# sujeetv/parquet-go

Measured on AMD Instinct MI355X. Metric: decoded GB/s (uncompressed output) per GPU & node at 1/2/4/8; % HBM roofline, higher is better.
Workload: dtype int32; 1 GPU; C2: optional INT32, 100000000 rows x 7 dictionary widths (b=1,2,4,8,12,16,20), ~10% nulls, RLE_DICTIONARY (uniform indices), V1, UNCOMPRESSED, 20000 rows/page; bytes_in=821696760, bytes_out=3220121800, streams=2, parallelism=single GPU

## Files before the change

### parquet-go_amd/csrc/pqg_lev1.h

```cpp
#pragma once
#include "pqg_levdec.h"

namespace pqg {

constexpr int kL1MaxN = 4096;
constexpr int kL1MaxCount = 32768 - 16;
constexpr int kL1Win = kL1MaxN + 64;
constexpr uint32_t kL1Far = 254, kL1Bad = 255;

struct Lev1Shared {
  uint8_t win[kL1Win];
  uint32_t tab[kL1MaxN / 4 + 2];
};

struct L1Hdr {
  uint32_t nx;
  uint32_t cnt;
  uint32_t pay;
  bool bp, bad;
};

__device__ __forceinline__ L1Hdr l1_hdr(uint32_t lo, uint32_t hi, uint32_t q, uint32_t n) {
  const uint32_t cont = ~lo & 0x80808080u;
  const uint32_t hl = (cont ? (uint32_t)__builtin_ctz(cont) >> 3 : 4u) + 1;
  const uint32_t hf = (lo & 0x7f) | ((lo >> 1) & 0x3f80) | ((lo >> 2) & 0x1fc000) | ((lo >> 3) & 0xfe00000);
  const uint32_t h = __builtin_amdgcn_ubfe(hf, 0, 7 * hl);
  const uint32_t g = h >> 1;
  const bool bp = (h & 1) != 0;
  const uint32_t vb = (uint32_t)((((uint64_t)hi << 32) | lo) >> (8 * hl)) & 0xff;
  const uint32_t ve = q + hl;
  L1Hdr r;
  r.bp = bp;
  r.bad = (hl > 4) | (ve > n) | (g == 0) | (!bp & ((ve >= n) | (vb > 1)));
  r.cnt = bp ? g * 8 : g;
  r.pay = bp ? ve : vb;
  r.nx = ve + (bp ? g : 1u);
  return r;
}
__device__ __forceinline__ L1Hdr l1_parse(const PQG_L uint8_t* win, uint32_t mis, uint32_t q, uint32_t n) {
  const uint32_t wo = mis + q;
  const PQG_L uint32_t* d = (const PQG_L uint32_t*)(win + (wo & ~3u));
  const uint32_t a = d[0], b = d[1], c = d[2];
  const uint32_t sft = (wo & 3) * 8;
  return l1_hdr(__builtin_amdgcn_alignbit(b, a, sft), __builtin_amdgcn_alignbit(c, b, sft), q, n);
}
struct L1Run {
  uint32_t hl, g, vb;
  bool bp;
};
__device__ __forceinline__ L1Run l1_run(const PQG_L uint8_t* win, uint32_t mis, uint32_t q) {
  const uint32_t wo = mis + q;
  const PQG_L uint32_t* d = (const PQG_L uint32_t*)(win + (wo & ~3u));
  const uint32_t a = d[0], b = d[1], c = d[2];
  const uint32_t sft = (wo & 3) * 8;
  const uint32_t lo = __builtin_amdgcn_alignbit(b, a, sft), hi = __builtin_amdgcn_alignbit(c, b, sft);
  const uint32_t cont = ~lo & 0x80808080u;
  L1Run r;
  r.hl = (cont ? (uint32_t)__builtin_ctz(cont) >> 3 : 3u) + 1;
  const uint32_t hf = (lo & 0x7f) | ((lo >> 1) & 0x3f80) | ((lo >> 2) & 0x1fc000) | ((lo >> 3) & 0xfe00000);
  const uint32_t h = __builtin_amdgcn_ubfe(hf, 0, 7 * r.hl);
  r.g = h >> 1;
  r.bp = (h & 1) != 0;
  r.vb = (uint32_t)((((uint64_t)hi << 32) | lo) >> (8 * r.hl)) & 0xff;
  return r;
}

__device__ __forceinline__ uint32_t l1_code(const L1Hdr& h, uint32_t e) {
  const uint32_t d = h.nx - e;
  return h.bad ? kL1Bad : (d < kL1Far ? d : kL1Far);
}

__device__ __forceinline__ void l1_or_run(PQG_L uint32_t* bm, const PQG_L uint32_t* W, uint32_t s, uint32_t len,
                                          bool bp, uint32_t sbit) {
  const uint32_t e = s + len;
  for (uint32_t k = s >> 5; 32 * k < e; k++) {
    const uint32_t lo = s > 32 * k ? s : 32 * k;
    const uint32_t hi = e < 32 * k + 32 ? e : 32 * k + 32;
    const uint32_t cnt = hi - lo;
    const uint32_t m = cnt >= 32 ? 0xffffffffu : ((1u << cnt) - 1);
    uint32_t v = m;
    if (bp) {
      const uint32_t sb = sbit + (lo - s);
      v = __builtin_amdgcn_alignbit(W[(sb >> 5) + 1], W[sb >> 5], sb & 31) & m;
    }
    v <<= (lo - 32 * k);
    if (v) __hip_atomic_fetch_or(bm + k, v, __ATOMIC_RELAXED, __HIP_MEMORY_SCOPE_WAVEFRONT);
  }
}

__device__ __forceinline__ bool lev1_page(gcu8 p, uint32_t n, uint32_t count, gu8 out, Lev1Shared& sh, uint32_t* nn_out) {
  const int lane = lane_id();
  if (n == 0 || n > (uint32_t)kL1MaxN || count > (uint32_t)kL1MaxCount) return false;
  PQG_L uint8_t* win = lds_ptr(sh.win);
  PQG_T(t0);
  const uintptr_t pa = (uintptr_t)p;
  const uint32_t mis = (uint32_t)(pa & 15);
  const uintptr_t base = pa - mis;
  const uint32_t lim = mis + n;
  constexpr int kR = (kL1Win + 1023) / 1024;
  uint4 v[kR];
#pragma unroll
  for (int h = 0; h < kR; h++) {
    const uint32_t g = 1024u * h + 16u * lane;
    v[h] = ldg16(g < lim ? base + g : base);
  }
#pragma unroll
  for (int h = 0; h < kR; h++) {
    const uint32_t g = 1024u * h + 16u * lane;
    if (g < (uint32_t)kL1Win) sts16(win + g, g < lim ? mask_tail(v[h], g, lim) : make_uint4(0, 0, 0, 0));
  }
  __builtin_amdgcn_wave_barrier();
  PQG_T(t1);
  PQG_ACC(20, t0, t1);
  PQG_L uint8_t* T = (PQG_L uint8_t*)lds_ptr(sh.tab);
  const uint32_t S = (((n + 63) >> 6) + 3) & ~3u;
  const uint32_t a = (uint32_t)lane * S;
  const uint32_t e = a + S < n ? a + S : n;
  int q = (int)e - 1;
  for (int r = (int)((e > a ? e - a : 0u) & 3); r > 0; r--, q--) {
    const L1Hdr h = l1_parse(win, mis, (uint32_t)q, n);
    uint32_t code = l1_code(h, e);
    if (!h.bad && h.nx < e) code = T[h.nx];
    T[q] = (uint8_t)code;
  }
  for (; q >= (int)a + 3; q -= 4) {
    const uint32_t q0 = (uint32_t)q - 3;
    const uint32_t wo = mis + q0;
    const PQG_L uint32_t* d = (const PQG_L uint32_t*)(win + (wo & ~3u));
    const uint32_t d0 = d[0], d1 = d[1], d2 = d[2], d3 = d[3];
    const uint32_t o = wo & 3;
    L1Hdr h[4];
#pragma unroll
    for (int j = 0; j < 4; j++) {
      const uint32_t oj = o + j;
      const uint32_t sft = (oj & 3) * 8;
      const bool up = oj >= 4;
      const uint32_t x0 = up ? d1 : d0, x1 = up ? d2 : d1, x2 = up ? d3 : d2;
      h[j] = l1_hdr(__builtin_amdgcn_alignbit(x1, x0, sft), __builtin_amdgcn_alignbit(x2, x1, sft), q0 + j, n);
    }
    uint32_t t[4], c[4];
    bool in[4];
#pragma unroll
    for (int j = 0; j < 4; j++) {
      in[j] = !h[j].bad & (h[j].nx < e);
      t[j] = T[in[j] ? h[j].nx : q0 + 3];
      c[j] = l1_code(h[j], e);
    }
    const uint32_t c3 = in[3] ? t[3] : c[3];
    const uint32_t c2 = in[2] ? t[2] : c[2];
    const uint32_t c1 = in[1] ? (h[1].nx == q0 + 3 ? c3 : t[1]) : c[1];
    const uint32_t c0 = in[0] ? (h[0].nx == q0 + 3 ? c3 : h[0].nx == q0 + 2 ? c2 : t[0]) : c[0];
    *(PQG_L uint32_t*)(T + q0) = c0 | c1 << 8 | c2 << 16 | c3 << 24;
  }
  __builtin_amdgcn_wave_barrier();
  PQG_T(t2);
  PQG_ACC(21, t1, t2);
  uint32_t E = 0, myE = 0;
  bool ok = true;
  for (int l = 0; l < 64; l++) {
    const uint32_t al = (uint32_t)l * S;
    if (lane == l) myE = E;
    if (al >= n) continue;
    const uint32_t el = al + S < n ? al + S : n;
    if (E >= el) continue;
    const uint32_t code = (uint32_t)__builtin_amdgcn_readfirstlane((int)T[E]);
    if (code == kL1Bad) { ok = false; break; }
    if (code == kL1Far) {
      uint32_t q = E;
      while (q < el) {
        const L1Hdr h = l1_parse(win, mis, q, n);
        if (h.bad) { ok = false; break; }
        q = (uint32_t)__builtin_amdgcn_readfirstlane((int)h.nx);
      }
      if (!ok) break;
      E = q;
    } else {
      E = el + code;
    }
  }
  PQG_T(t3);
  PQG_ACC(22, t2, t3);
  if (!ok) { PQG_ACC(27, 0, 1); return false; }
#ifdef PQG_L1_STOP_AFTER_LINK
  *nn_out = 0;
  return true;
#endif
  uint32_t C = 0;
  uint64_t cm = 0;
  for (uint32_t q = myE; q < e;) {
    const L1Run r = l1_run(win, mis, q);
    const uint32_t cnt = r.bp ? r.g * 8 : r.g;
    C = C + cnt < (1u << 24) ? C + cnt : (1u << 24);
    cm |= 1ull << (q - a);
    q += r.hl + (r.bp ? r.g : 1u);
  }
  const uint32_t incl = ldpp_incl_add_sat(C);
  const uint32_t total = (uint32_t)__builtin_amdgcn_readlane((int)incl, 63);
  if (total < count) return false;
  const uint32_t B = incl - C;
  PQG_T(t4);
  PQG_ACC(23, t3, t4);
  const uintptr_t oa = (uintptr_t)out;
  const uintptr_t a0 = oa & ~(uintptr_t)15;
  const uint32_t pre = (uint32_t)(oa - a0);
  const uint32_t end = pre + count;
  PQG_L uint32_t* bm = lds_ptr(sh.tab);
  const uint32_t nw = (end + 31) >> 5;
  __builtin_amdgcn_wave_barrier();
  for (uint32_t k = (uint32_t)lane; k <= nw; k += 64) bm[k] = 0u;
  __builtin_amdgcn_wave_barrier();
  const PQG_L uint32_t* W = (const PQG_L uint32_t*)win;
  bool fail = false;
  uint32_t c = B;
  uint32_t k = (pre + c) >> 5, fill = (pre + c) & 31;
  uint64_t acc = 0;
  const uint32_t kfirst = k;
  uint32_t nn = 0;
  uint64_t m = c < count ? cm : 0ull;
#ifdef PQG_L1_SKIP_EMIT
  m = 0;
#endif
  auto flush = [&](uint32_t word) {
    if (k == kfirst) __hip_atomic_fetch_or(bm + k, word, __ATOMIC_RELAXED, __HIP_MEMORY_SCOPE_WAVEFRONT);
    else bm[k] = word;
    nn += __builtin_popcount(word);
    k++;
  };
  uint32_t rq = 0;
  L1Run r{};
  if (m) {
    rq = a + (uint32_t)__builtin_ctzll(m);
    m &= m - 1;
    r = l1_run(win, mis, rq);
  }
  bool more = c < count && cm != 0;
  while (more) {
    const L1Run cur = r;
    const uint32_t cq = rq;
    const bool next = m != 0;
    if (next) {
      rq = a + (uint32_t)__builtin_ctzll(m);
      m &= m - 1;
      r = l1_run(win, mis, rq);
    }
    const uint32_t cnt = cur.bp ? cur.g * 8 : cur.g;
    uint32_t take = cnt < count - c ? cnt : count - c;
    const uint32_t pay = cq + cur.hl;
    if (cur.bp && pay + ((take + 7) >> 3) - 1 >= n) { fail = true; break; }
    c += take;
    const uint32_t pat = cur.vb ? 0xffffffffu : 0u;
    const bool bp = cur.bp;
    uint32_t sb = bp ? (mis + pay) * 8 : 0u;
    while (take) {
      const uint32_t nb = take < 32 ? take : 32;
      const uint32_t src = __builtin_amdgcn_alignbit(W[(sb >> 5) + 1], W[sb >> 5], sb & 31);
      const uint32_t bits = (bp ? src : pat) & (nb >= 32 ? 0xffffffffu : ((1u << nb) - 1));
      acc |= (uint64_t)bits << fill;
      fill += nb;
      take -= nb;
      sb += nb;
      if (fill >= 32) {
        flush((uint32_t)acc);
        acc >>= 32;
        fill -= 32;
      }
    }
    more = next && c < count;
  }
  if (fill) {
    __hip_atomic_fetch_or(bm + k, (uint32_t)acc, __ATOMIC_RELAXED, __HIP_MEMORY_SCOPE_WAVEFRONT);
    nn += __builtin_popcount((uint32_t)acc);
  }
  if (__ballot(fail)) return false;
  PQG_T(t5);
  PQG_ACC(24, t4, t5);
  __builtin_amdgcn_wave_barrier();
  const PQG_L uint16_t* B16 = (const PQG_L uint16_t*)lds_ptr(sh.tab);
#ifdef PQG_L1_SKIP_EXPAND
  const uint32_t g0 = 1, g1 = 0;
#else
  const uint32_t g0 = (pre + 15) >> 4, g1 = end >> 4;
#endif
  for (uint32_t g = g0 + (uint32_t)lane; g < g1; g += 64) {
    const uint32_t b16 = B16[g];
    uint32_t wv[4];
#pragma unroll
    for (int j = 0; j < 4; j++) wv[j] = (((b16 >> (4 * j)) & 0xfu) * 0x00204081u) & 0x01010101u;
    stg16o(a0 + 16 * g, make_uint4(wv[0], wv[1], wv[2], wv[3]));
  }
  if (lane < 32) {
    const uint32_t gr = lane < 16 ? (pre >> 4) : (end >> 4);
    const uint32_t i = 16 * gr + (uint32_t)(lane & 15);
    if (i >= pre && i < end && (i < 16 * g0 || i >= 16 * g1))
      *(PQG_G uint8_t*)(a0 + i) = (uint8_t)((B16[gr] >> (lane & 15)) & 1);
  }
  *nn_out = (uint32_t)wave_sum((int64_t)nn);
  PQG_T(t6);
  PQG_ACC(25, t5, t6);
  PQG_ACC(26, 0, 1);
  return true;
}

}
```

Baseline: 1428 GB/s.

## SWAR-parse four RLE level headers per word and flatten emit loop

Replaces the four per-byte level header parses in the backward jump-table pass with a SIMD-within-a-register routine. It decodes four candidate headers at once from packed bytes, derives their lengths, bad/far flags and codes with byte-lane arithmetic, and treats headers longer than two bytes as 'far' for the slow path. It also flattens the nested run/chunk loops of the bitmap emit phase into a single loop that refills runs on demand, and moves the parser into a shared host/device header. The aim is fewer ALU ops and less branch divergence in definition-level decoding, at the cost of more intricate bit logic and extra tail handling near the page end.

```diff
diff --git a/parquet-go_amd/csrc/pqg_lev1.h b/parquet-go_amd/csrc/pqg_lev1.h
--- a/parquet-go_amd/csrc/pqg_lev1.h
+++ b/parquet-go_amd/csrc/pqg_lev1.h
@@ -1,42 +1,18 @@
 #pragma once
 #include "pqg_levdec.h"
+#include "pqg_lev1_parse.h"
 
 namespace pqg {
 
 constexpr int kL1MaxN = 4096;
 constexpr int kL1MaxCount = 32768 - 16;
 constexpr int kL1Win = kL1MaxN + 64;
-constexpr uint32_t kL1Far = 254, kL1Bad = 255;
 
 struct Lev1Shared {
   uint8_t win[kL1Win];
   uint32_t tab[kL1MaxN / 4 + 2];
 };
 
-struct L1Hdr {
-  uint32_t nx;
-  uint32_t cnt;
-  uint32_t pay;
-  bool bp, bad;
-};
-
-__device__ __forceinline__ L1Hdr l1_hdr(uint32_t lo, uint32_t hi, uint32_t q, uint32_t n) {
-  const uint32_t cont = ~lo & 0x80808080u;
-  const uint32_t hl = (cont ? (uint32_t)__builtin_ctz(cont) >> 3 : 4u) + 1;
-  const uint32_t hf = (lo & 0x7f) | ((lo >> 1) & 0x3f80) | ((lo >> 2) & 0x1fc000) | ((lo >> 3) & 0xfe00000);
-  const uint32_t h = __builtin_amdgcn_ubfe(hf, 0, 7 * hl);
-  const uint32_t g = h >> 1;
-  const bool bp = (h & 1) != 0;
-  const uint32_t vb = (uint32_t)((((uint64_t)hi << 32) | lo) >> (8 * hl)) & 0xff;
-  const uint32_t ve = q + hl;
-  L1Hdr r;
-  r.bp = bp;
-  r.bad = (hl > 4) | (ve > n) | (g == 0) | (!bp & ((ve >= n) | (vb > 1)));
-  r.cnt = bp ? g * 8 : g;
-  r.pay = bp ? ve : vb;
-  r.nx = ve + (bp ? g : 1u);
-  return r;
-}
 __device__ __forceinline__ L1Hdr l1_parse(const PQG_L uint8_t* win, uint32_t mis, uint32_t q, uint32_t n) {
   const uint32_t wo = mis + q;
   const PQG_L uint32_t* d = (const PQG_L uint32_t*)(win + (wo & ~3u));
@@ -70,24 +46,6 @@
   return h.bad ? kL1Bad : (d < kL1Far ? d : kL1Far);
 }
 
-__device__ __forceinline__ void l1_or_run(PQG_L uint32_t* bm, const PQG_L uint32_t* W, uint32_t s, uint32_t len,
-                                          bool bp, uint32_t sbit) {
-  const uint32_t e = s + len;
-  for (uint32_t k = s >> 5; 32 * k < e; k++) {
-    const uint32_t lo = s > 32 * k ? s : 32 * k;
-    const uint32_t hi = e < 32 * k + 32 ? e : 32 * k + 32;
-    const uint32_t cnt = hi - lo;
-    const uint32_t m = cnt >= 32 ? 0xffffffffu : ((1u << cnt) - 1);
-    uint32_t v = m;
-    if (bp) {
-      const uint32_t sb = sbit + (lo - s);
-      v = __builtin_amdgcn_alignbit(W[(sb >> 5) + 1], W[sb >> 5], sb & 31) & m;
-    }
-    v <<= (lo - 32 * k);
-    if (v) __hip_atomic_fetch_or(bm + k, v, __ATOMIC_RELAXED, __HIP_MEMORY_SCOPE_WAVEFRONT);
-  }
-}
-
 __device__ __forceinline__ bool lev1_page(gcu8 p, uint32_t n, uint32_t count, gu8 out, Lev1Shared& sh, uint32_t* nn_out) {
   const int lane = lane_id();
   if (n == 0 || n > (uint32_t)kL1MaxN || count > (uint32_t)kL1MaxCount) return false;
@@ -117,7 +75,11 @@
   const uint32_t a = (uint32_t)lane * S;
   const uint32_t e = a + S < n ? a + S : n;
   int q = (int)e - 1;
-  for (int r = (int)((e > a ? e - a : 0u) & 3); r > 0; r--, q--) {
+  const uint32_t len = e > a ? e - a : 0u;
+  uint32_t top = len & 3;
+  if (e - top + 3 > n) top += 4;
+  top = top < len ? top : len;
+  for (int r = (int)top; r > 0; r--, q--) {
     const L1Hdr h = l1_parse(win, mis, (uint32_t)q, n);
     uint32_t code = l1_code(h, e);
     if (!h.bad && h.nx < e) code = T[h.nx];
@@ -127,30 +89,24 @@
     const uint32_t q0 = (uint32_t)q - 3;
     const uint32_t wo = mis + q0;
     const PQG_L uint32_t* d = (const PQG_L uint32_t*)(win + (wo & ~3u));
-    const uint32_t d0 = d[0], d1 = d[1], d2 = d[2], d3 = d[3];
-    const uint32_t o = wo & 3;
-    L1Hdr h[4];
+    const uint32_t d0 = d[0], d1 = d[1], d2 = d[2];
+    const uint32_t sft = (wo & 3) * 8;
+    const uint32_t b0 = __builtin_amdgcn_alignbit(d1, d0, sft), b4 = __builtin_amdgcn_alignbit(d2, d1, sft);
+    const L1Quad h = l1_quad(b0, __builtin_amdgcn_alignbit(b4, b0, 8), __builtin_amdgcn_alignbit(b4, b0, 16));
+    const L1Codes cd = l1_quad_codes(h, e - q0);
+    const uint32_t in7 = cd.in, code = cd.code;
+    const uint32_t inm = in7 | (in7 - (in7 >> 7));
+    uint32_t nx[4], t[4];
 #pragma unroll
     for (int j = 0; j < 4; j++) {
-      const uint32_t oj = o + j;
-      const uint32_t sft = (oj & 3) * 8;
-      const bool up = oj >= 4;
-      const uint32_t x0 = up ? d1 : d0, x1 = up ? d2 : d1, x2 = up ? d3 : d2;
-      h[j] = l1_hdr(__builtin_amdgcn_alignbit(x1, x0, sft), __builtin_amdgcn_alignbit(x2, x1, sft), q0 + j, n);
-    }
-    uint32_t t[4], c[4];
-    bool in[4];
-#pragma unroll
-    for (int j = 0; j < 4; j++) {
-      in[j] = !h[j].bad & (h[j].nx < e);
-      t[j] = T[in[j] ? h[j].nx : q0 + 3];
-      c[j] = l1_code(h[j], e);
-    }
-    const uint32_t c3 = in[3] ? t[3] : c[3];
-    const uint32_t c2 = in[2] ? t[2] : c[2];
-    const uint32_t c1 = in[1] ? (h[1].nx == q0 + 3 ? c3 : t[1]) : c[1];
-    const uint32_t c0 = in[0] ? (h[0].nx == q0 + 3 ? c3 : h[0].nx == q0 + 2 ? c2 : t[0]) : c[0];
-    *(PQG_L uint32_t*)(T + q0) = c0 | c1 << 8 | c2 << 16 | c3 << 24;
+      nx[j] = q0 + j + ((h.len >> (8 * j)) & 0xff);
+      t[j] = T[(in7 >> (8 * j + 7)) & 1 ? nx[j] : q0 + 3];
+    }
+    const uint32_t up = (code & ~inm) | ((t[2] << 16 | t[3] << 24) & inm);
+    const uint32_t c3 = up >> 24, c2 = (up >> 16) & 0xff;
+    const uint32_t t1 = nx[1] == q0 + 3 ? c3 : t[1];
+    const uint32_t t0 = nx[0] == q0 + 3 ? c3 : nx[0] == q0 + 2 ? c2 : t[0];
+    *(PQG_L uint32_t*)(T + q0) = up | ((t0 | t1 << 8) & inm);
   }
   __builtin_amdgcn_wave_barrier();
   PQG_T(t2);
@@ -228,46 +184,45 @@
   };
   uint32_t rq = 0;
   L1Run r{};
-  if (m) {
+  bool have = m != 0;
+  if (have) {
     rq = a + (uint32_t)__builtin_ctzll(m);
     m &= m - 1;
     r = l1_run(win, mis, rq);
   }
-  bool more = c < count && cm != 0;
-  while (more) {
-    const L1Run cur = r;
-    const uint32_t cq = rq;
-    const bool next = m != 0;
-    if (next) {
-      rq = a + (uint32_t)__builtin_ctzll(m);
-      m &= m - 1;
-      r = l1_run(win, mis, rq);
-    }
-    const uint32_t cnt = cur.bp ? cur.g * 8 : cur.g;
-    uint32_t take = cnt < count - c ? cnt : count - c;
-    const uint32_t pay = cq + cur.hl;
-    if (cur.bp && pay + ((take + 7) >> 3) - 1 >= n) { fail = true; break; }
-    c += take;
-    const uint32_t pat = cur.vb ? 0xffffffffu : 0u;
-    const bool bp = cur.bp;
-    uint32_t sb = bp ? (mis + pay) * 8 : 0u;
-    while (take) {
-      const uint32_t nb = take < 32 ? take : 32;
-      const uint32_t src = __builtin_amdgcn_alignbit(W[(sb >> 5) + 1], W[sb >> 5], sb & 31);
-      const uint32_t bits = (bp ? src : pat) & (nb >= 32 ? 0xffffffffu : ((1u << nb) - 1));
-      acc |= (uint64_t)bits << fill;
-      fill += nb;
-      take -= nb;
-      sb += nb;
-      if (fill >= 32) {
-        flush((uint32_t)acc);
-        acc >>= 32;
-        fill -= 32;
+  uint32_t take = 0, sb = 0, pat = 0;
+  bool bp = false;
+  while (have | (take != 0)) {
+    if (take == 0) {
+      const uint32_t cnt = r.bp ? r.g * 8 : r.g;
+      take = cnt < count - c ? cnt : count - c;
+      const uint32_t pay = rq + r.hl;
+      if (r.bp && pay + ((take + 7) >> 3) - 1 >= n) { fail = true; break; }
+      c += take;
+      have = m != 0 && c < count;
+      pat = r.vb ? 0xffffffffu : 0u;
+      bp = r.bp;
+      sb = bp ? (mis + pay) * 8 : 0u;
+      if (have) {
+        rq = a + (uint32_t)__builtin_ctzll(m);
+        m &= m - 1;
+        r = l1_run(win, mis, rq);
       }
     }
-    more = next && c < count;
-  }
-  if (fill) {
+    const uint32_t nb = take < 32 ? take : 32;
+    const uint32_t src = __builtin_amdgcn_alignbit(W[(sb >> 5) + 1], W[sb >> 5], sb & 31);
+    const uint32_t bits = (bp ? src : pat) & (nb >= 32 ? 0xffffffffu : ((1u << nb) - 1));
+    acc |= (uint64_t)bits << fill;
+    fill += nb;
+    take -= nb;
+    sb += nb;
+    if (fill >= 32) {
+      flush((uint32_t)acc);
+      acc >>= 32;
+      fill -= 32;
+    }
+  }
+  if (fill && B < count) {
     __hip_atomic_fetch_or(bm + k, (uint32_t)acc, __ATOMIC_RELAXED, __HIP_MEMORY_SCOPE_WAVEFRONT);
     nn += __builtin_popcount((uint32_t)acc);
   }
diff --git a/parquet-go_amd/csrc/pqg_lev1_parse.h b/parquet-go_amd/csrc/pqg_lev1_parse.h
--- /dev/null
+++ b/parquet-go_amd/csrc/pqg_lev1_parse.h
@@ -0,0 +1,87 @@
+#pragma once
+#include <cstdint>
+
+#if defined(__HIPCC__)
+#define PQG_HD __host__ __device__ __forceinline__
+#else
+#define PQG_HD inline
+#endif
+
+namespace pqg {
+
+constexpr uint32_t kL1Far = 254, kL1Bad = 255;
+
+struct L1Hdr {
+  uint32_t nx;
+  uint32_t cnt;
+  uint32_t pay;
+  bool bp, bad;
+};
+
+PQG_HD L1Hdr l1_hdr(uint32_t lo, uint32_t hi, uint32_t q, uint32_t n) {
+  const uint32_t cont = ~lo & 0x80808080u;
+  const uint32_t hl = (cont ? (uint32_t)__builtin_ctz(cont) >> 3 : 4u) + 1;
+  const uint32_t hf = (lo & 0x7f) | ((lo >> 1) & 0x3f80) | ((lo >> 2) & 0x1fc000) | ((lo >> 3) & 0xfe00000);
+#if defined(__HIP_DEVICE_COMPILE__)
+  const uint32_t h = __builtin_amdgcn_ubfe(hf, 0, 7 * hl);
+#else
+  const uint32_t h = hl > 4 ? hf : hf & ((1u << (7 * hl)) - 1);
+#endif
+  const uint32_t g = h >> 1;
+  const bool bp = (h & 1) != 0;
+  const uint32_t vb = (uint32_t)((((uint64_t)hi << 32) | lo) >> (8 * hl)) & 0xff;
+  const uint32_t ve = q + hl;
+  L1Hdr r;
+  r.bp = bp;
+  r.bad = (hl > 4) | (ve > n) | (g == 0) | ((!bp) & ((ve >= n) | (vb > 1)));
+  r.cnt = bp ? g * 8 : g;
+  r.pay = bp ? ve : vb;
+  r.nx = ve + (bp ? g : 1u);
+  return r;
+}
+
+struct L1Quad {
+  uint32_t len, bad, far;
+};
+PQG_HD uint32_t l1q_nz(uint32_t x) {
+  return ((x & 0x7f7f7f7fu) + 0x7f7f7f7fu) | x;
+}
+PQG_HD L1Quad l1_quad(uint32_t b0, uint32_t b1, uint32_t b2) {
+  constexpr uint32_t H = 0x80808080u, L7 = 0x7f7f7f7fu, O = 0x01010101u;
+  const uint32_t c0 = b0 & H;
+  const uint32_t two = c0 & ~b1;
+  const uint32_t far3 = c0 & b1;
+  const uint32_t m2 = two | (two - (two >> 7));
+  const uint32_t bpm = (b0 & O) * 0xffu;
+  const uint32_t low = (b0 >> 1) & 0x3f3f3f3fu;
+  const uint32_t b1m = b1 & m2;
+  const uint32_t gm = low | ((b1m & 0x03030303u) << 6);
+  const uint32_t gz = ~l1q_nz(low | b1m);
+  const uint32_t big = l1q_nz(b1m & 0x7c7c7c7cu) | ~l1q_nz(~gm & 0xfcfcfcfcu);
+  const uint32_t vb = (b2 & m2) | (b1 & ~m2);
+  const uint32_t vbig = l1q_nz(vb & 0xfefefefeu);
+  L1Quad r;
+  r.far = (far3 | (big & bpm)) & H;
+  r.bad = (gz | (vbig & ~bpm)) & ~r.far & H;
+  const uint32_t x = (gm & bpm) | (O & ~bpm);
+  r.len = (((x & L7) + O + (two >> 7)) ^ (x & H));
+  return r;
+}
+
+
+struct L1Codes {
+  uint32_t code, in;
+};
+PQG_HD L1Codes l1_quad_codes(const L1Quad& h, uint32_t ed) {
+  constexpr uint32_t H = 0x80808080u;
+  const uint32_t dist = ed * 0x01010101u - 0x03020100u;
+  const uint32_t df = (h.len | H) - dist;
+  const uint32_t fb = h.far | h.bad;
+  const uint32_t fbm = fb | (fb - (fb >> 7));
+  L1Codes r;
+  r.in = ~h.len & ~df & ~fb & H;
+  r.code = ((df ^ (~h.len & H)) & ~fbm) | (fbm ^ (h.far >> 7));
+  return r;
+}
+
+}
```

Measured after the change: 1477 GB/s (median of 6 runs). 1.03x the previous value.
